# openclimatefix/skillful_nowcasting

Hardware: AMD Instinct MI355X
Metric: radar frames/sec (G+D step) 4->18 @256^2 (higher is better)
Workload: dtype mixed (fp32 tensors + accumulate; bf16x3 = 2 bf16 planes, 3 MFMAs/product, 16-bit products; discriminator forward bf16x6); 1 GPU; DGMR.training_step paper: forecast_steps=18, output_shape=256, latent_channels=768, context_channels=384, generation_steps=6, H=W=256; per_gpu_batch=16, global_batch=16, parallelism=dp1

## Files before the change

skillful_nowcasting_amd/csrc/conv.hip:

```cpp
#include <cstdlib>
#include <cstring>
#include <map>
#include <mutex>
#include <string>
#include <vector>

#include "conv_bf16.h"
#include "conv_device.h"
#include "conv_launch.h"
#include "conv_stem4.h"

namespace {

template <int BM, int BN, int BK, int WM, int WN>
__global__ __launch_bounds__(64 * WM * WN) void conv_igemm_kernel(const dgmr_conv_args p, const int M, const int Ktot,
                                                                   const int kt_per_split) {
    constexpr int NT = 64 * WM * WN;
    constexpr int LD = BK + 4;
    constexpr int KQ = BK / 4;
    constexpr int RPP = NT / KQ;
    constexpr int AP = BM / RPP, BP = BN / RPP;
    constexpr int TM = BM / WM / 32, TN = BN / WN / 32;
    static_assert(AP >= 1 && BP >= 1 && TM >= 1 && TN >= 1, "bad tile");
    static_assert(BM % RPP == 0 && BN % RPP == 0, "bad tile");
// ... 1013 lines not shown
    float a = 0.f;
    if (c < Cout) {
        int r = l;
        for (; r + 28 < nrows; r += 32) {
            float v[8];
#pragma unroll
            for (int k = 0; k < 8; ++k) v[k] = rows[(size_t)(r + 4 * k) * Cout + c];
#pragma unroll
            for (int k = 0; k < 8; ++k) a += v[k];
        }
        for (; r < nrows; r += 4) a += rows[(size_t)r * Cout + c];
    }
    part[l][col] = a;
    __syncthreads();
    if (l == 0 && c < Cout) bias_grad[c] += (part[0][col] + part[1][col]) + (part[2][col] + part[3][col]);
}
static inline int colsum_rows_for(int64_t M) { return (int)std::max<int64_t>(1, std::min<int64_t>(1024, M / 512)); }

static bool wgrad_ws() { return g_tune_wgrad_window != 1; }
static const bool g_wgrad_psplit = []() {
    const char* e = getenv("DGMR_WGRAD_PSPLIT");
    return !(e && e[0] == '0');
}();
static bool wgrad_uses_window(const dgmr_wgrad_args* a) {
    const bool k2d = a->KD == 1 && a->D == 1, k3d = a->KD == 3 && a->D >= 1 && !a->upsample && wgrad_ws();
    return g_precision != 0 && g_tune_wgrad_window != 0 && (k2d || k3d) && a->KH == 3 && a->KW == 3 &&
           ((a->W % 32 == 0 && a->H % 2 == 0) || (a->W == 16 && a->H % 4 == 0));
}
static int wgrad_window_tw_shift(const dgmr_wgrad_args* a) { return a->W % 32 == 0 ? 5 : 4; }
static const bool g_wgrad_phases = []() {
    const char* e = getenv("DGMR_WGRAD_PHASES");
    return !(e && e[0] == '0');
}();
static bool wgrad_by_phases(const dgmr_wgrad_args* a) {
    if (!((g_tune_wgrad_window == 4 || (g_tune_wgrad_window < 0 && g_wgrad_phases)) && a->upsample && a->KD == 1 && a->D == 1 && a->KH == 3 && a->KW == 3 &&
          (g_precision == 1 || g_precision == 2) && a->H % 2 == 0 && a->W % 2 == 0))
        return false;
    const int h = a->H / 2, w = a->W / 2;
    return (w % 32 == 0 && h % 2 == 0) || (w == 16 && h % 4 == 0);
}

extern "C" int dgmr_conv_wgrad_plan(dgmr_wgrad_args* a) {
    DGMR_CHECK_ARG(a && a->N > 0 && a->Cin > 0 && a->Cout > 0, "dgmr_conv_wgrad_plan: bad args");
    const int groups = a->groups < 1 ? 1 : a->groups;
    DGMR_CHECK_ARG(a->N % groups == 0, "dgmr_conv_wgrad_plan: N=%d not divisible by groups=%d", a->N, groups);
    const int64_t M = (int64_t)a->N * a->D * a->H * a->W;
    if (!wgrad_uses_window(a)) {
        a->nsplit = dgmr_conv_wgrad_nsplit((int)M, a->Cout, a->KD * a->KH * a->KW * a->Cin, groups);
        a->bias_rows = std::max(a->nsplit, colsum_rows_for(M));
        return 0;
    }
    const int per_slab = ((a->Cin + 31) / 32) * (a->Cout % 96 == 0 ? a->Cout / 96 : (a->Cout + 63) / 64);
    const bool phases = wgrad_by_phases(a);
    const int64_t tiles_per_group = (int64_t)(a->N / groups) * a->D * ((int64_t)a->H * a->W / (phases ? 256 : 64));
    int64_t per = 512 / ((int64_t)per_slab * groups);
    per = std::min<int64_t>(per, tiles_per_group / 2);
    per = std::max<int64_t>(per, 1);
    if (wgrad_ws()) per = std::max<int64_t>(1, std::min<int64_t>(256 / ((int64_t)per_slab * groups), tiles_per_group / 2));
    a->nsplit = (int)std::min<int64_t>(per * groups, 4096) * (phases ? 4 : 1);
    a->bias_rows = std::max(a->nsplit, colsum_rows_for(M));
    return 0;
}

extern "C" int dgmr_conv_wgrad(const dgmr_wgrad_args* a, void* stream) {
    DGMR_CHECK_ARG(a && a->x && a->dy && a->partial, "dgmr_conv_wgrad: null pointer");
    DGMR_CHECK_ARG(a->Cin % 4 == 0 && a->Cout % 4 == 0, "dgmr_conv_wgrad: Cin=%d Cout=%d must be multiples of 4", a->Cin,
                   a->Cout);
    DGMR_CHECK_ARG(a->nsplit >= 1, "dgmr_conv_wgrad: nsplit=%d", a->nsplit);
// ... 11 lines not shown
    DGMR_CHECK_ARG(!bias_rows_mode || a->bias_rows >= std::max(a->nsplit, colsum_rows_for(M64)),
                   "dgmr_conv_wgrad: bias_rows=%d (dgmr_conv_wgrad_plan fills it in)", a->bias_rows);
    hipStream_t s_ = (hipStream_t)stream;
    auto bias_rows_begin = [&](int rows) { (void)hipMemsetAsync(a->bias_partial, 0, sizeof(float) * (size_t)rows * a->Cout, s_); };
    auto bias_rows_finish = [&](int rows) {
        hipLaunchKernelGGL(bias_rows_finish_kernel, dim3((a->Cout + 63) / 64), dim3(256), 0, s_, a->bias_partial, rows, a->Cout, a->bias_grad);
    };
    auto bias_by_colsum = [&]() {
        const int rows = colsum_rows_for(M64);
        hipLaunchKernelGGL(colsum_rows_kernel, dim3(rows), dim3(256), 0, s_, a->dy, a->bias_partial, M64, a->Cout, rows);
        bias_rows_finish(rows);
    };
    const int M = (int)M64, Ktot = a->KD * a->KH * a->KW * a->Cin;
    const int spg = a->nsplit / groups, rows_per_group = M / groups;
    int rows = (rows_per_group + spg - 1) / spg;
    rows = (rows + 31) / 32 * 32;
    hipStream_t s = (hipStream_t)stream;
    const int kt = (Ktot + 127) / 128;
    const int wclass = a->Cout <= 32 ? V_W32 : (a->Cout <= 64 ? V_W64 : V_W128);
    const uint32_t wdetail = 3u | ((wgrad_uses_window(a) ? (wgrad_ws() ? 2u : 1u) : 0u) << 4) | ((uint32_t)(wclass - V_W128) << 6) |
                             ((a->KD == 3 ? 1u : 0u) << 8) | ((a->upsample ? 1u : 0u) << 9) | ((Ktot == a->Cin ? 1u : 0u) << 10);
    ProfScope ps(wclass, 2.0 * (double)M64 * (double)Ktot * (double)a->Cout, s, 1.0, wdetail);
    if (wgrad_uses_window(a) && wgrad_by_phases(a) && a->nsplit % (4 * groups) == 0) {
        dgmr_wgrad_args q = p;
        q.H = a->H / 2, q.W = a->W / 2, q.upsample = 0;
        const int spg4 = a->nsplit / 4 / groups;
        const int tw_shift = wgrad_window_tw_shift(&q);
        const int tiles_w = q.W >> tw_shift, tiles_hw = (q.H / (64 >> tw_shift)) * tiles_w;
        const int tiles_per_group = (a->N / groups) * tiles_hw;
        const int tiles_per_split = (tiles_per_group + spg4 - 1) / spg4;
        const bool b96 = a->Cout % 96 == 0;
        const dim3 grid((a->Cin + 31) / 32, b96 ? a->Cout / 96 : (a->Cout + 63) / 64, a->nsplit / 4);
        if (bias_rows_mode) bias_rows_begin(a->nsplit);
        for (int ph = 0; ph < 4; ++ph) {
            if (bias_rows_mode) q.bias_grad = a->bias_partial + (size_t)ph * (a->nsplit / 4) * a->Cout, q.bias_stride = a->Cout;
            DGMR_BY_NS(launch_wgrad_window, q, grid, tw_shift, tiles_w, tiles_hw, tiles_per_split, spg4, tiles_per_group,
                       1 | ((g_debug_flags & 16) >> 3) | 4 | 8 | (ph << 16), s);
            DGMR_CHECK_LAUNCH();
        }
        if (bias_rows_mode) bias_rows_finish(a->nsplit);
        return 0;
    }
    if (wgrad_uses_window(a)) {
        const int tw_shift = wgrad_window_tw_shift(a);
        const int tiles_w = a->W >> tw_shift, tiles_hw = (a->H / (64 >> tw_shift)) * tiles_w;
        const int tiles_per_group = (a->N / groups) * a->D * tiles_hw;
        const int tiles_per_split = (tiles_per_group + spg - 1) / spg;
        const bool b96 = a->Cout % 96 == 0;
        const dim3 grid((a->Cin + 31) / 32, b96 ? a->Cout / 96 : (a->Cout + 63) / 64, a->nsplit);
        const bool rows_in_kernel = bias_rows_mode && wgrad_ws();
        if (rows_in_kernel) bias_rows_begin(a->nsplit);
        for (int kd = 0; kd < a->KD; ++kd) {
            dgmr_wgrad_args q = p;
            if (a->KD == 3 && kd != 1) q.bias_grad = nullptr;
            else if (rows_in_kernel) q.bias_grad = a->bias_partial, q.bias_stride = a->Cout;
            else if (bias_rows_mode) q.bias_grad = nullptr;
            DGMR_BY_NS(launch_wgrad_window, q, grid, tw_shift, tiles_w, tiles_hw, tiles_per_split, spg, tiles_per_group,
                       wgrad_ws() ? (1 | ((g_debug_flags & 16) >> 3) | (g_tune_wgrad_window != 2 && g_precision != 3 ? 4 : 0) | ((g_tune_wgrad_window == 5 || !g_wgrad_psplit) ? 32 : 0) | (kd << 8)) : 0, s);
            DGMR_CHECK_LAUNCH();
        }
        if (rows_in_kernel) bias_rows_finish(a->nsplit);
        else if (bias_rows_mode) bias_by_colsum();
        return 0;
    }
    if (bias_rows_mode && g_precision != 0) {
        bias_rows_begin(a->nsplit);
        p.bias_grad = a->bias_partial, p.bias_stride = a->Cout;
    } else if (bias_rows_mode) {
        p.bias_grad = nullptr;
    }
// ... 161 lines not shown
    DGMR_CHECK_LAUNCH();
    return 0;
}

extern "C" int dgmr_split_weights(const float* w, uint16_t* out, int64_t rows, int Cin, int w_cin, int w_coff, int planes,
                                  int64_t plane_stride, void* stream) {
    DGMR_CHECK_ARG(w && out && rows > 0 && Cin > 0 && Cin % 2 == 0, "dgmr_split_weights: bad args (Cin=%d must be even)", Cin);
    DGMR_CHECK_ARG(planes >= 1 && planes <= 3, "dgmr_split_weights: planes=%d (1 .. 3)", planes);
    if (w_cin == 0) {
        w_cin = Cin;
        w_coff = 0;
    }
    DGMR_CHECK_ARG(w_coff >= 0 && w_coff + Cin <= w_cin, "dgmr_split_weights: bad slice");
    const int64_t total = rows * Cin;
    if (plane_stride == 0) plane_stride = total;
    DGMR_CHECK_ARG(plane_stride >= total && plane_stride % 2 == 0, "dgmr_split_weights: plane_stride=%lld < %lld elements", (long long)plane_stride,
                   (long long)total);
    const int blocks = (int)std::min<int64_t>((total / 2 + 255) / 256, 2048);
    hipLaunchKernelGGL(split_weights_kernel, dim3(blocks), dim3(256), 0, (hipStream_t)stream, w, out, total, Cin, w_cin, w_coff, planes,
                       plane_stride);
    DGMR_CHECK_LAUNCH();
    return 0;
}

extern "C" int dgmr_set_precision(int mode) {
    DGMR_CHECK_ARG(mode >= 0 && mode <= 3, "dgmr_set_precision: mode %d (0 f32, 1 bf16x3, 2 bf16, 3 bf16x6)", mode);
    g_precision = mode;
    return 0;
}
extern "C" int dgmr_get_precision(void) { return g_precision; }

extern "C" int dgmr_conv_tune(int variant, int ksplit, int window, int wgrad_window) {
    DGMR_CHECK_ARG(variant >= -1 && variant <= V_F128x32 && ksplit >= -1 && window >= -1 && window <= 7 && wgrad_window >= -1 &&
                       wgrad_window <= 5,
                   "dgmr_conv_tune: variant %d ksplit %d window %d wgrad_window %d", variant, ksplit, window, wgrad_window);
    g_tune_variant = variant;
    g_tune_ksplit = ksplit;
    g_tune_window = window;
    g_tune_wgrad_window = wgrad_window;
    return 0;
}

extern "C" int dgmr_debug_flags(int flags) {
    DGMR_CHECK_ARG(flags >= 0 && flags <= 8191 && !(flags & 4), "dgmr_debug_flags: %d", flags);
    g_debug_flags = flags;
    return 0;
}

extern "C" int dgmr_profile_enable(int on) {
    std::lock_guard<std::mutex> lk(g_prof_mu);
    g_prof_on = on != 0;
    return 0;
}

extern "C" int dgmr_profile_variants(void) { return V_COUNT; }
extern "C" const char* dgmr_profile_variant_name(int v) { return (v >= 0 && v < V_COUNT) ? kVariantNames[v] : ""; }

extern "C" int dgmr_profile_collect(double* total_ms, double* total_flops, int64_t* launches, int n) {
    return dgmr_profile_collect2(total_ms, total_flops, nullptr, launches, n);
}

static std::string prof_detail_name(int variant, uint32_t d) {
    static const char* const prec[] = {"f32", "bf16x3", "bf16", "bf16x6"};
    char b[160];
    const int kind = d & 15;
    const char* pr = prec[(d >> 28) & 3];
    if (kind == 1) {
        static const int bn[] = {48, 64, 96, 128, 16, 0, 0, 0};
        static const char* const mode[] = {"plain", "phase", "pooled", "phase4"};
        snprintf(b, sizeof b, "win3x3<bn%d,%dpx>%s%s%s%s %s %s", bn[(d >> 4) & 7], (d >> 8) & 1 ? 256 : 128, (d >> 13) & 1 ? " reg-staged" : "",
                 (d >> 11) & 1 ? " 3d" : "", (d >> 14) & 1 ? " gru" : "", (d >> 15) & 1 ? " ws" : "", mode[(d >> 9) & 3], (d >> 12) & 1 ? "small(<1024wg)" : "big");
    } else if (kind == 2) {
        snprintf(b, sizeof b, "%s%s%s%s%s %s", kVariantNames[variant], (d >> 8) & 1 ? " splitk" : "", (d >> 9) & 1 ? " 1x1" : "",
                 (d >> 11) & 1 ? " 3d" : "", (d >> 14) & 1 ? " gru" : "", (d >> 12) & 1 ? "small(<1024wg)" : "big");
    } else if (kind == 5) {
        snprintf(b, sizeof b, "conv1x1 stream (%s class)", kVariantNames[variant]);
    } else if (kind == 4) {
// ... 60 lines not shown
```

skillful_nowcasting_amd/csrc/conv_launch.h:

```cpp
#pragma once
#include "common.h"

#define DGMR_HIDDEN __attribute__((visibility("hidden")))

enum { V_F128x128 = 0, V_F64x64, V_F128x96, V_F128x64, V_F128x32, V_W128, V_W64, V_W32, V_WIN128, V_WIN96, V_WIN64, V_COUNT };

struct WinPlan {
    int tw_shift, g_shift, tiles_w, tiles_hw, bnw, grid_x;
    bool big, glds;
    bool ws;
    int ws_ups;
    bool pair;
};

namespace dgmr_tu {

inline int ns_of_precision(int prec) { return prec == 1 ? 3 : (prec == 2 ? 1 : 6); }

#define DGMR_TU_DECLARE(NS)                                                                                                          \
    DGMR_HIDDEN int launch_window_ns##NS(const dgmr_conv_args& p, const WinPlan& wp, bool phases, int tune_window, hipStream_t s);   \
    DGMR_HIDDEN int launch_gemm_ns##NS(int variant, const dgmr_conv_args& p, int M, int Ktot, int kt_per_split, dim3 grid,           \
                                       hipStream_t s);                                                                               \
    DGMR_HIDDEN int launch_wgrad_window_ns##NS(const dgmr_wgrad_args& p, dim3 grid, int tw_shift, int tiles_w, int tiles_hw,         \
                                               int tiles_per_split, int splits_per_group, int tiles_per_group, int ws,         \
                                               hipStream_t s);                                                                        \
    DGMR_HIDDEN int launch_wgrad_gemm_ns##NS(const dgmr_wgrad_args& p, int bi, dim3 grid, int M, int Ktot, int rows_per_split,       \
                                             int splits_per_group, int rows_per_group, hipStream_t s);
DGMR_TU_DECLARE(1)
DGMR_TU_DECLARE(3)
DGMR_TU_DECLARE(6)
#undef DGMR_TU_DECLARE
DGMR_HIDDEN int launch_conv1x1_ns1(const dgmr_conv_args& p, int M, int rows_per_sample, hipStream_t s);
DGMR_HIDDEN int launch_conv1x1_ns3(const dgmr_conv_args& p, int M, int rows_per_sample, hipStream_t s);

#define DGMR_TU_DECLARE_WS(NS, MODE) \
    DGMR_HIDDEN int launch_window_ws_ns##NS##_m##MODE(const dgmr_conv_args& p, const WinPlan& wp, int grid, hipStream_t s);
DGMR_TU_DECLARE_WS(1, 0)
DGMR_TU_DECLARE_WS(1, 1)
DGMR_TU_DECLARE_WS(1, 2)
DGMR_TU_DECLARE_WS(3, 0)
DGMR_TU_DECLARE_WS(3, 1)
DGMR_TU_DECLARE_WS(3, 2)
#undef DGMR_TU_DECLARE_WS

}

#define DGMR_TU_CAT_(a, b) a##b
#define DGMR_TU_CAT(a, b) DGMR_TU_CAT_(a, b)
```

skillful_nowcasting_amd/csrc/tu_wgrad.hip:

```cpp
#include "conv_launch.h"
#include "wgrad_win.h"
#include "wgrad_ws.h"

#ifndef DGMR_NS
#error "compile with -DDGMR_NS=1|3|6"
#endif

namespace dgmr_tu {

int DGMR_TU_CAT(launch_wgrad_window_ns, DGMR_NS)(const dgmr_wgrad_args& p, dim3 grid, int tw_shift, int tiles_w, int tiles_hw,
                                                 int tiles_per_split, int splits_per_group, int tiles_per_group, int ws, hipStream_t s) {
    constexpr int NS = DGMR_NS;
    const bool b96 = p.Cout % 96 == 0;
    if (ws) {
#define DGMR_WGS(BI_, TWS_)                                                                                                      \
    do {                                                                                                                         \
        if constexpr (NS != 6) {                                                                                                 \
            if (ws & 8) {                  \
                hipLaunchKernelGGL((conv_wgrad_ws_kernel<BI_, NS, TWS_, 4, true>), dim3(grid.x * grid.y * grid.z), dim3(512), 0, s, p,     \
                                   tiles_w, tiles_hw, tiles_per_split, splits_per_group, tiles_per_group, ws & 0xff, 0, (ws >> 16) & 3, 4); \
                break;                                                                                                           \
            }                                                                                                                    \
            if (ws & 4) {                                                                                                        \
                hipLaunchKernelGGL((conv_wgrad_ws_kernel<BI_, NS, TWS_, 4>), dim3(grid.x * grid.y * grid.z), dim3(512), 0, s, p, tiles_w, \
                                   tiles_hw, tiles_per_split, splits_per_group, tiles_per_group, ws & 0xff, (ws >> 8) & 0xff);   \
                break;                                                                                                           \
            }                                                                                                                    \
        }                                                                                                                        \
        hipLaunchKernelGGL((conv_wgrad_ws_kernel<BI_, NS, TWS_, 3>), dim3(grid.x * grid.y * grid.z), dim3(448), 0, s, p, tiles_w,    \
                           tiles_hw, tiles_per_split, splits_per_group, tiles_per_group, ws & 0xff, (ws >> 8) & 0xff);           \
    } while (0)
        bool done = false;
        if constexpr (NS != 6) {
            if (p.Cout <= 48 && (ws & 4) && !(ws & 8) && !(ws & 32)) {
                if (tw_shift == 5)
                    hipLaunchKernelGGL((conv_wgrad_ws_kernel<48, NS, 5, 4, false, true>), dim3(grid.x * grid.y * grid.z), dim3(512), 0, s, p, tiles_w,
                                       tiles_hw, tiles_per_split, splits_per_group, tiles_per_group, ws & 0x1f, (ws >> 8) & 0xff);
                else
                    hipLaunchKernelGGL((conv_wgrad_ws_kernel<48, NS, 4, 4, false, true>), dim3(grid.x * grid.y * grid.z), dim3(512), 0, s, p, tiles_w,
                                       tiles_hw, tiles_per_split, splits_per_group, tiles_per_group, ws & 0x1f, (ws >> 8) & 0xff);
                done = true;
            }
        }
        if (done) return 0;
        if (b96) {
            if (tw_shift == 5) DGMR_WGS(96, 5);
            else DGMR_WGS(96, 4);
        } else {
            if (tw_shift == 5) DGMR_WGS(64, 5);
            else DGMR_WGS(64, 4);
// ... 33 lines not shown
```

skillful_nowcasting_amd/csrc/wgrad_ws.h:

```cpp
#pragma once
#include "conv_bf16.h"

namespace {

typedef short s16x4 __attribute__((ext_vector_type(4)));
typedef short s16x8 __attribute__((ext_vector_type(8)));
typedef __attribute__((address_space(3))) s16x4 lds_s16x4;

__device__ __forceinline__ s16x4 lds_read_tr(const uint32_t* p) {
#if defined(__HIP_DEVICE_COMPILE__)
    return __builtin_amdgcn_ds_read_tr16_b64_v4i16((lds_s16x4*)p);
#else
    (void)p;
    return (s16x4){0, 0, 0, 0};
#endif
}
__device__ __forceinline__ bf16x8_t tr_fragment(const uint32_t* p, int row4_dwords) {
    const s16x4 lo = lds_read_tr(p), hi = lds_read_tr(p + row4_dwords);
    const s16x8 v = {lo[0], lo[1], lo[2], lo[3], hi[0], hi[1], hi[2], hi[3]};
    return __builtin_bit_cast(bf16x8_t, v);
}

constexpr int ws_gcd(int a, int b) { return b == 0 ? a : ws_gcd(b, a % b); }

template <int READS, int M, int I>
__device__ __forceinline__ void ws_interleave() {
    if constexpr (I < M) {
        __builtin_amdgcn_sched_group_barrier(0x008, 1, 0);
        constexpr int N = (READS * (I + 1)) / M - (READS * I) / M;
        if constexpr (N > 0) __builtin_amdgcn_sched_group_barrier(0x100, N, 0);
        ws_interleave<READS, M, I + 1>();
    }
}

template <int BI, int NS, int TWS, int MW = 3, bool PHASE = false, bool PSPLIT = false>
__global__ __launch_bounds__(MW * 64 + 256) void conv_wgrad_ws_kernel(const dgmr_wgrad_args p, const int tiles_w, const int tiles_hw,
                                                           const int tiles_per_split, const int splits_per_group,
                                                           const int tiles_per_group, const int dbg, const int kd, const int ph = 0,
                                                           const int slab_mul = 1) {
    static_assert(!PHASE || MW == 4, "phase mode: four matrix waves");
    const int ppy = PHASE ? ph >> 1 : 0, ppx = PHASE ? ph & 1 : 0;
    constexpr int NP = planes_of<NS>::value;
    constexpr int CK = 32, CB = BI / 32;
    constexpr int TW = 1 << TWS, TH = 64 >> TWS;
    constexpr int HTW = TW + 2, HTH = TH + 2;
    constexpr int HPIX = HTH * HTW;
    constexpr int XROW = CK / 2;
    constexpr int YROW = 48;
    constexpr int XPL = HPIX * XROW, YPL = MW == 4 ? 64 * (BI / 2) : 64 * YROW;
    constexpr int BUF = NP * (XPL + YPL);
    constexpr int NL = 256;
    constexpr int XITEMS = HPIX * 8, YQ = BI / 4, YITEMS = 64 * YQ;
    constexpr int XP = (XITEMS + NL - 1) / NL, YP = YITEMS / NL;
    constexpr int BSN = NL % YQ == 0 ? 1 : YQ / ws_gcd(NL % YQ, YQ);
    static_assert(BI == 64 || BI == 96 || (BI == 48 && PSPLIT), "BI");
    static_assert(!PSPLIT || (MW == 4 && !PHASE && BI == 48 && NP <= 2), "pixel-split tile");
    constexpr int NACC4 = 9 * 3 * 4;
    constexpr int RED_DW = ((NL % (BI / 4) == 0 ? 1 : (BI / 4) / ws_gcd(NL % (BI / 4), BI / 4)) * NL * 4);
    constexpr int EXCH_DW = PSPLIT ? 2 * NACC4 * 64 : 0;
    static_assert(TWS == 5 || TWS == 4, "tile width");
    static_assert(YITEMS % NL == 0 && YP % BSN == 0, "dY items per loader thread");

    __shared__ __attribute__((aligned(16))) uint32_t smem[(2 * BUF > RED_DW + EXCH_DW) ? 2 * BUF : RED_DW + EXCH_DW];

    const int tid = threadIdx.x, lane = tid & 63;
    const int wid = __builtin_amdgcn_readfirstlane(tid >> 6);
    const int n_chunks = (p.Cin + CK - 1) / CK, n_cot = (p.Cout + BI - 1) / BI;
    const int total = gridDim.x, xcd = blockIdx.x & 7, per_xcd = total >> 3, rem = total & 7;
    const int wg = xcd * per_xcd + min(xcd, rem) + (blockIdx.x >> 3);
    const int chunk = wg % n_chunks, wg2 = wg / n_chunks;
    const int slab = wg2 / n_cot, co0 = (wg2 - slab * n_cot) * BI;
    const int grp = slab / splits_per_group;
    const int t_begin = grp * tiles_per_group + (slab - grp * splits_per_group) * tiles_per_split;
    const int t_end = min((grp + 1) * tiles_per_group, t_begin + tiles_per_split);
    const int nt = max(t_end - t_begin, 0);
    const bool want_bias = p.bias_grad && chunk == 0;
    float* red = reinterpret_cast<float*>(smem);

    if (wid >= MW) {
        const int lt = tid - MW * 64;
        const int xq = lt & 7;
        const int xci = chunk * CK + xq * 4;
        const bool xc_ok = xci < p.Cin;
        const int us = (!PHASE && p.upsample) ? 1 : 0;
        const int Hs = p.H >> us, Ws = p.W >> us;
        const f32x4 zero4 = {0.f, 0.f, 0.f, 0.f};
        int xrel[XP];
        uint32_t yrel[YP];
        unsigned m_all = 0, m_top = 0, m_bot = 0, m_left = 0, m_right = 0, y_ok = 0;
#pragma unroll
        for (int i = 0; i < XP; ++i) {
            const int idx = lt + i * NL;
            const int pix = idx >> 3;
            const int pr = pix / HTW, pc = pix - pr * HTW;
            xrel[i] = (((pr - 1) >> us) * Ws + ((pc - 1) >> us)) * p.Cin + xci;
            const unsigned bit = 1u << i;
            m_all |= (idx < XITEMS && xc_ok) ? bit : 0u;
            m_top |= pr == 0 ? bit : 0u;
            m_bot |= pr == HTH - 1 ? bit : 0u;
            m_left |= pc == 0 ? bit : 0u;
            m_right |= pc == HTW - 1 ? bit : 0u;
        }
#pragma unroll
        for (int i = 0; i < YP; ++i) {
            const int idx = lt + i * NL;
            const int pix = idx / YQ, q = idx - pix * YQ;
            const int co = co0 + q * 4;
            yrel[i] = PHASE ? (uint32_t)((pix >> TWS) * 4 * p.W + (pix & (TW - 1)) * 2) * p.Cout + min(co, p.Cout - 4)
                            : (uint32_t)((pix >> TWS) * p.W + (pix & (TW - 1))) * p.Cout + min(co, p.Cout - 4);
            y_ok |= co < p.Cout ? 1u << i : 0u;
        }
        int cn = t_begin / tiles_hw, ch0, cw0, left = nt - 1;
        {
            const int trem = t_begin - cn * tiles_hw;
            const int th = trem / tiles_w;
            ch0 = th * TH;
            cw0 = (trem - th * tiles_w) << TWS;
        }
        const int Dp = p.D, dshift = p.KD == 3 ? kd - 1 : 0;
        int cd = cn % Dp;
        const float relu_floor = (p.pre_a || p.pre_relu) ? 0.f : -__builtin_inff();
        f32x4 sx[2][XP], sy[2][YP], sa[2], sb[2], bsum[BSN];
        unsigned xm[2] = {0, 0};
#pragma unroll
        for (int e = 0; e < 2; ++e) sa[e] = (f32x4){1.f, 1.f, 1.f, 1.f}, sb[e] = zero4;
#pragma unroll
        for (int i = 0; i < BSN; ++i) bsum[i] = zero4;

        auto issue = [&](auto set_c) {
            constexpr int E = decltype(set_c)::value;
            const uint32_t xb = (((uint32_t)(cn + dshift) * Hs + (ch0 >> us)) * Ws + (cw0 >> us)) * p.Cin;
            const bool plane_ok = (unsigned)(cd + dshift) < (unsigned)Dp;
            const unsigned kill = (ch0 == 0 ? m_top : 0u) | (ch0 + TH >= p.H ? m_bot : 0u) | (cw0 == 0 ? m_left : 0u) | (cw0 + TW >= p.W ? m_right : 0u);
            const unsigned m = plane_ok ? m_all & ~kill : 0u;
            xm[E] = m;
#pragma unroll
            for (int i = 0; i < XP; ++i) sx[E][i] = *reinterpret_cast<const f32x4*>(p.x + (((m >> i) & 1u) ? xb + (uint32_t)xrel[i] : 0u));
            if (p.pre_a) {
                const uint32_t g = xc_ok ? (uint32_t)(cn / Dp / p.pre_group) * p.Cin + xci : 0u;
                sa[E] = *reinterpret_cast<const f32x4*>(p.pre_a + g);
                sb[E] = *reinterpret_cast<const f32x4*>(p.pre_b + g);
            }
            const float* yb = PHASE ? p.dy + (((size_t)cn * 2 * p.H + 2 * ch0 + ppy) * 2 * p.W + 2 * cw0 + ppx) * p.Cout
                                    : p.dy + (((size_t)cn * p.H + ch0) * p.W + cw0) * p.Cout;
#pragma unroll
            for (int i = 0; i < YP; ++i) sy[E][i] = *reinterpret_cast<const f32x4*>(yb + yrel[i]);
            if (left > 0) {
                --left;
                cw0 += TW;
                if (cw0 >= p.W) {
                    cw0 = 0;
                    ch0 += TH;
                    if (ch0 >= p.H) {
                        ch0 = 0;
                        ++cn;
                        cd = cd + 1 == Dp ? 0 : cd + 1;
                    }
                }
            }
        };
        auto store = [&](auto set_c, bool live) {
            constexpr int E = decltype(set_c)::value;
            uint32_t* Xs = smem + E * BUF + (MW == 4 ? (xq >> 2) * (HPIX * 8) + (lt >> 3) * 8 + (xq & 3) * 2 : lt * 2);
            uint32_t* Ys = smem + E * BUF + NP * XPL;
            const unsigned m = xm[E];
#pragma unroll
            for (int i = 0; i < XP; ++i) {
                if (i == XP - 1 && XITEMS % NL != 0 && lt + i * NL >= XITEMS) continue;
                f32x4 v = sx[E][i];
#pragma unroll
                for (int c = 0; c < 4; ++c) v[c] = fmaxf(fmaf(v[c], sa[E][c], sb[E][c]), relu_floor);
                v = ((m >> i) & 1u) ? v : zero4;
                u32x2 pl[NP];
                split_planes4<NP>(v, pl);
#pragma unroll
                for (int q = 0; q < NP; ++q) *reinterpret_cast<u32x2*>(Xs + q * XPL + i * (MW == 4 ? NL : NL * 2)) = pl[q];
            }
#pragma unroll
            for (int i = 0; i < YP; ++i) {
                const int idx = lt + i * NL;
                const int pix = idx / YQ, q = idx - pix * YQ;
                const f32x4 v = ((y_ok >> i) & 1u) ? sy[E][i] : zero4;
                if (want_bias && live) bsum[i % BSN] += v;
                u32x2 pl[NP];
                split_planes4<NP>(v, pl);
#pragma unroll
                for (int k = 0; k < NP; ++k)
                    *reinterpret_cast<u32x2*>(Ys + k * YPL + (MW == 4 ? (q >> 2) * (64 * 8) + pix * 8 + (q & 3) * 2 : pix * YROW + q * 2)) = pl[k];
            }
        };
        using set0 = std::integral_constant<int, 0>;
        using set1 = std::integral_constant<int, 1>;
        if (nt > 0) {
            issue(set0{});
            issue(set1{});
            store(set0{}, true);
            issue(set0{});
            __syncthreads();
            for (int t = 0; t < nt; t += 2) {
                store(set1{}, t + 1 < nt);
                issue(set1{});
                __syncthreads();
                store(set0{}, t + 2 < nt);
                issue(set0{});
                __syncthreads();
            }
        } else {
            __syncthreads();
        }
        if (want_bias) {
#pragma unroll
            for (int i = 0; i < BSN; ++i) *reinterpret_cast<f32x4*>(red + (i * NL + lt) * 4) = bsum[i];
        }
        if (want_bias || PSPLIT) __syncthreads();
    } else {
        if constexpr (MW == 4) {
            constexpr int CBH = PSPLIT ? 3 : BI / 32;
            const int cih = wid & 1, coh = PSPLIT ? 0 : wid >> 1;
            const int psh = PSPLIT ? wid >> 1 : 0;
            constexpr int NT = PHASE ? 4 : 9;
            f32x4 acc[NT][CBH];
#pragma unroll
            for (int t = 0; t < NT; ++t)
#pragma unroll
                for (int c = 0; c < CBH; ++c) acc[t][c] = (f32x4){0.f, 0.f, 0.f, 0.f};
            const int tg = lane >> 4, ti = lane & 15;
            const int py_lane = 16 * (tg >> 1) + 4 * (tg & 1) + (ti >> 2);
            const int px_lane = (TWS == 5 ? 16 * (tg >> 1) : (tg >> 1) * HTW) + 4 * (tg & 1) + (ti >> 2);
            const int seg = (ti & 3) * 2;
            auto compute = [&](int buf) {
                const uint32_t* Xs = smem + buf * BUF + cih * (HPIX * 8) + px_lane * 8 + seg;
                const uint32_t* Ys = smem + buf * BUF + NP * XPL + coh * CBH * (64 * 8) + py_lane * 8 + seg;
                auto fetch_x = [&](int ks, int pl, bf16x8_t (&dst)[NT]) {
#pragma unroll
                    for (int t = 0; t < NT; ++t) {
                        const int hp = PHASE ? ((TWS == 5 ? ks : 2 * ks) + ppy + (t >> 1)) * HTW + ppx + (t & 1)
                                             : ((TWS == 5 ? ks : 2 * ks) + t / 3) * HTW + t % 3;
                        dst[t] = tr_fragment(Xs + pl * XPL + hp * 8, 8 * 8);
                    }
                };
                auto fetch_y = [&](int ks, int pl, bf16x8_t (&dst)[CBH]) {
#pragma unroll
                    for (int c = 0; c < CBH; ++c) dst[c] = tr_fragment(Ys + pl * YPL + c * (64 * 8) + ks * 32 * 8, 8 * 8);
                };
                auto mm = [&](const bf16x8_t (&y)[CBH], const bf16x8_t (&x)[NT]) {
#pragma unroll
                    for (int t = 0; t < NT; ++t)
#pragma unroll
                        for (int c = 0; c < CBH; ++c) acc[t][c] = __builtin_amdgcn_mfma_f32_16x16x32_bf16(y[c], x[t], acc[t][c], 0, 0, 0);
                };
                constexpr int M = NT * CBH, RX = 2 * NT, RY = CBH * 2, RX0 = PHASE ? 4 : 6;
                if constexpr (PSPLIT) {
                    if constexpr (NP == 2) {
                        bf16x8_t y0[CBH], y1[CBH], x0[NT], x1[NT];
                        fetch_y(psh, 0, y0), fetch_x(psh, 1, x1);
                        __builtin_amdgcn_sched_group_barrier(0x100, RY + RX0, 0);
                        fetch_y(psh, 1, y1), fetch_x(psh, 0, x0);
                        mm(y0, x1);
                        ws_interleave<RX - RX0 + RX + RY, M, 0>();
                        mm(y1, x0);
                        __builtin_amdgcn_sched_group_barrier(0x008, M, 0);
                        mm(y0, x0);
                        __builtin_amdgcn_sched_group_barrier(0x008, M, 0);
                    } else {
                        bf16x8_t xf[NT], yf[CBH];
                        fetch_y(psh, 0, yf), fetch_x(psh, 0, xf);
                        mm(yf, xf);
                    }
                } else if constexpr (NP == 2) {
                    bf16x8_t y0[2][CBH], x0[NT], x1[NT], y1[CBH];
                    fetch_y(0, 0, y0[0]), fetch_x(0, 1, x1);
                    __builtin_amdgcn_sched_group_barrier(0x100, RY + RX0, 0);
#pragma unroll
                    for (int ks = 0; ks < 2; ++ks) {
                        const int e = ks & 1;
                        fetch_y(ks, 1, y1), fetch_x(ks, 0, x0);
                        mm(y0[e], x1);
                        if (ks == 0) ws_interleave<RX - RX0 + RX + RY, M, 0>();
                        else ws_interleave<RX + RY, M, 0>();
                        if (ks < 1) fetch_x(ks + 1, 1, x1), fetch_y(ks + 1, 0, y0[e ^ 1]);
                        mm(y1, x0);
                        if (ks < 1) ws_interleave<RX + RY, M, 0>();
                        else __builtin_amdgcn_sched_group_barrier(0x008, M, 0);
                        mm(y0[e], x0);
                        __builtin_amdgcn_sched_group_barrier(0x008, M, 0);
                    }
                } else {
                    static_assert(NP == 1, "four matrix waves: bf16 and bf16x3 only (bf16x6 needs 144 fragment registers)");
                    bf16x8_t xf[2][NT], yf[2][CBH];
                    fetch_y(0, 0, yf[0]), fetch_x(0, 0, xf[0]);
                    fetch_y(1, 0, yf[1]), fetch_x(1, 0, xf[1]);
                    mm(yf[0], xf[0]);
                    mm(yf[1], xf[1]);
                }
            };
            __builtin_amdgcn_s_setprio(1);
            __syncthreads();
            for (int t = 0; t < nt; t += 2) {
                if (!(dbg & 2)) compute(0);
                __syncthreads();
                if (t + 1 < nt && !(dbg & 2)) compute(1);
                __syncthreads();
            }
            if constexpr (PSPLIT) {
                float* ex = reinterpret_cast<float*>(smem) + RED_DW + cih * (NACC4 * 64) + lane;
                if (psh == 1) {
#pragma unroll
                    for (int t = 0; t < NT; ++t)
#pragma unroll
                        for (int c = 0; c < CBH; ++c)
#pragma unroll
                            for (int r = 0; r < 4; ++r) ex[((t * CBH + c) * 4 + r) * 64] = acc[t][c][r];
                }
                __syncthreads();
                if (psh == 0) {
#pragma unroll
                    for (int t = 0; t < NT; ++t)
#pragma unroll
                        for (int c = 0; c < CBH; ++c)
#pragma unroll
                            for (int r = 0; r < 4; ++r) acc[t][c][r] += ex[((t * CBH + c) * 4 + r) * 64];
                }
            }
            const int Ktot = 9 * p.KD * p.Cin, tap0 = (p.KD == 3 ? kd : 0) * 9;
            float* out = p.partial + ((size_t)slab * slab_mul + (PHASE ? ph : 0)) * p.Cout * Ktot;
            const int ci = chunk * CK + cih * 16 + (lane & 15);
            if (ci < p.Cin && psh == 0) {
#pragma unroll
                for (int c = 0; c < CBH; ++c)
#pragma unroll
                    for (int r = 0; r < 4; ++r) {
                        const int co = co0 + (coh * CBH + c) * 16 + 4 * (lane >> 4) + r;
                        if (co >= p.Cout) continue;
#pragma unroll
                        for (int t = 0; t < 9; ++t) {
                            float v;
                            if constexpr (PHASE) {
                                const int a = (t / 3 + 1 - ppy) >> 1, b = (t % 3 + 1 - ppx) >> 1;
                                const float va0 = b ? acc[1][c][r] : acc[0][c][r], va1 = b ? acc[3][c][r] : acc[2][c][r];
                                v = a ? va1 : va0;
                            } else {
                                v = acc[t][c][r];
                            }
                            out[(size_t)co * Ktot + (tap0 + t) * p.Cin + ci] = v;
                        }
                    }
            }
        } else {
            f32x16 acc[CB * 3];
    #pragma unroll
            for (int a = 0; a < CB * 3; ++a)
    #pragma unroll
                for (int r = 0; r < 16; ++r) acc[a][r] = 0.f;
            const int tg = lane >> 4, ti = lane & 15;
            const int k_lane = 8 * (tg >> 1) + (ti >> 2);
            const int col_lane = 16 * (tg & 1) + 4 * (ti & 3);
            auto compute = [&](int buf) {
                const uint32_t* Xs = smem + buf * BUF;
                const uint32_t* Ys = Xs + NP * XPL;
                auto fetch_x = [&](int kk, int pl, bf16x8_t (&dst)[3]) {
                    const int hp0 = (((kk * 16) >> TWS) + wid) * HTW + ((kk * 16) & (TW - 1));
                    const uint32_t* xb = Xs + pl * XPL + (hp0 + k_lane) * XROW + (col_lane >> 1);
    #pragma unroll
                    for (int d = 0; d < 3; ++d) dst[d] = tr_fragment(xb + d * XROW, 4 * XROW);
                };
                auto fetch_y = [&](int kk, int pl, bf16x8_t (&dst)[CB]) {
                    const uint32_t* yb = Ys + pl * YPL + (kk * 16 + k_lane) * YROW + (col_lane >> 1);
    #pragma unroll
                    for (int c = 0; c < CB; ++c) dst[c] = tr_fragment(yb + c * 16, 4 * YROW);
                };
                auto mm = [&](const bf16x8_t (&y)[CB], const bf16x8_t (&x)[3]) {
    #pragma unroll
                    for (int c = 0; c < CB; ++c)
    #pragma unroll
                        for (int d = 0; d < 3; ++d) acc[c * 3 + d] = __builtin_amdgcn_mfma_f32_32x32x16_bf16(y[c], x[d], acc[c * 3 + d], 0, 0, 0);
                };
                auto interleave = [&](auto reads_c) { ws_interleave<decltype(reads_c)::value, CB * 3, 0>(); };
                if constexpr (NP == 2) {
                    constexpr int RX = 3 * 2, RY = CB * 2;
// ... 29 lines not shown
    #pragma unroll
                        for (int pl = 0; pl < NP; ++pl) fetch_x(kk, pl, xf[pl]), fetch_y(kk, pl, yf[pl]);
                        for_each_product<NP>([&](auto qa, auto qb) { mm(yf[qa], xf[qb]); });
                    }
                }
            };
            __builtin_amdgcn_s_setprio(1);
            __syncthreads();
            for (int t = 0; t < nt; t += 2) {
                if (!(dbg & 2)) compute(0);
                __syncthreads();
                if (t + 1 < nt && !(dbg & 2)) compute(1);
                __syncthreads();
            }
            const int Ktot = 9 * p.KD * p.Cin, tap0 = (p.KD == 3 ? kd : 0) * 9;
            float* out = p.partial + (size_t)slab * p.Cout * Ktot;
            const int ci = chunk * CK + (lane & 31);
            if (ci < p.Cin) {
    #pragma unroll
                for (int c = 0; c < CB; ++c)
    #pragma unroll
                    for (int r = 0; r < 16; ++r) {
                        const int co = co0 + c * 32 + (r & 3) + 8 * (r >> 2) + 4 * (lane >> 5);
                        if (co >= p.Cout) continue;
    #pragma unroll
                        for (int d = 0; d < 3; ++d) out[(size_t)co * Ktot + (tap0 + wid * 3 + d) * p.Cin + ci] = acc[c * 3 + d][r];
                    }
            }
        }
        if (want_bias) {
            if (!PSPLIT) __syncthreads();
            if (tid < BI && co0 + tid < p.Cout) {
                const int q = tid >> 2, comp = tid & 3;
                float total = 0.f;
#pragma unroll
                for (int i = 0; i < BSN; ++i)
                    for (int l = ((q - i * NL) % YQ + YQ) % YQ; l < NL; l += YQ) total += red[(i * NL + l) * 4 + comp];
                atomicAdd(p.bias_grad + (size_t)slab * p.bias_stride + co0 + tid, total);
            }
        }
    }
}

}
```

Baseline: 463.5 radar frames/s.

## Pair column-parity phases in upsample wgrad window kernel to share X tile

For the phase-decomposed weight gradient of upsampled 3x3 convolutions, one launch now handles both column parities of a row phase. The kernel loads the shared input X tile once, stages two dY images, keeps two accumulator sets, and writes both phase outputs and bias partials. This halves the launches (four down to two) and the X loads and plane splitting they repeat. In exchange it doubles dY shared memory, accumulator registers and reduction space, which may lower occupancy. It is on by default through an env flag, and tune value 6 disables the pairing.

```diff
diff --git a/skillful_nowcasting_amd/csrc/conv.hip b/skillful_nowcasting_amd/csrc/conv.hip
--- a/skillful_nowcasting_amd/csrc/conv.hip
+++ b/skillful_nowcasting_amd/csrc/conv.hip
@@ -1069,8 +1069,13 @@
     const char* e = getenv("DGMR_WGRAD_PHASES");
     return !(e && e[0] == '0');
 }();
+static const bool g_wgrad_phase_pair = []() {
+    const char* e = getenv("DGMR_WGRAD_PHASE_PAIR");
+    return !(e && e[0] == '0');
+}();
 static bool wgrad_by_phases(const dgmr_wgrad_args* a) {
-    if (!((g_tune_wgrad_window == 4 || (g_tune_wgrad_window < 0 && g_wgrad_phases)) && a->upsample && a->KD == 1 && a->D == 1 && a->KH == 3 && a->KW == 3 &&
+    const bool tuned = g_tune_wgrad_window == 4 || g_tune_wgrad_window == 6;
+    if (!((tuned || (g_tune_wgrad_window < 0 && g_wgrad_phases)) && a->upsample && a->KD == 1 && a->D == 1 && a->KH == 3 && a->KW == 3 &&
           (g_precision == 1 || g_precision == 2) && a->H % 2 == 0 && a->W % 2 == 0))
         return false;
     const int h = a->H / 2, w = a->W / 2;
@@ -1148,10 +1153,13 @@
         const bool b96 = a->Cout % 96 == 0;
         const dim3 grid((a->Cin + 31) / 32, b96 ? a->Cout / 96 : (a->Cout + 63) / 64, a->nsplit / 4);
         if (bias_rows_mode) bias_rows_begin(a->nsplit);
-        for (int ph = 0; ph < 4; ++ph) {
-            if (bias_rows_mode) q.bias_grad = a->bias_partial + (size_t)ph * (a->nsplit / 4) * a->Cout, q.bias_stride = a->Cout;
+        const bool pair = g_tune_wgrad_window == 4 || (g_tune_wgrad_window < 0 && g_wgrad_phase_pair);
+        const int parity_rows = (a->nsplit / 4) * a->Cout;
+        for (int ph = 0; ph < 4; ph += pair ? 2 : 1) {
+            if (pair && ph && (g_debug_flags & 8192)) break;
+            if (bias_rows_mode) q.bias_grad = a->bias_partial + (size_t)ph * parity_rows, q.bias_stride = a->Cout;
             DGMR_BY_NS(launch_wgrad_window, q, grid, tw_shift, tiles_w, tiles_hw, tiles_per_split, spg4, tiles_per_group,
-                       1 | ((g_debug_flags & 16) >> 3) | 4 | 8 | (ph << 16), s);
+                       1 | ((g_debug_flags & 16) >> 3) | 4 | 8 | (ph << 16) | (pair ? 1 << 18 : 0), s, bias_rows_mode ? parity_rows : 0);
             DGMR_CHECK_LAUNCH();
         }
         if (bias_rows_mode) bias_rows_finish(a->nsplit);
@@ -1379,7 +1387,7 @@
 
 extern "C" int dgmr_conv_tune(int variant, int ksplit, int window, int wgrad_window) {
     DGMR_CHECK_ARG(variant >= -1 && variant <= V_F128x32 && ksplit >= -1 && window >= -1 && window <= 7 && wgrad_window >= -1 &&
-                       wgrad_window <= 5,
+                       wgrad_window <= 6,
                    "dgmr_conv_tune: variant %d ksplit %d window %d wgrad_window %d", variant, ksplit, window, wgrad_window);
     g_tune_variant = variant;
     g_tune_ksplit = ksplit;
@@ -1389,7 +1397,7 @@
 }
 
 extern "C" int dgmr_debug_flags(int flags) {
-    DGMR_CHECK_ARG(flags >= 0 && flags <= 8191 && !(flags & 4), "dgmr_debug_flags: %d", flags);
+    DGMR_CHECK_ARG(flags >= 0 && flags <= 16383 && !(flags & 4), "dgmr_debug_flags: %d", flags);
     g_debug_flags = flags;
     return 0;
 }
diff --git a/skillful_nowcasting_amd/csrc/conv_launch.h b/skillful_nowcasting_amd/csrc/conv_launch.h
--- a/skillful_nowcasting_amd/csrc/conv_launch.h
+++ b/skillful_nowcasting_amd/csrc/conv_launch.h
@@ -23,7 +23,7 @@
                                        hipStream_t s);                                                                               \
     DGMR_HIDDEN int launch_wgrad_window_ns##NS(const dgmr_wgrad_args& p, dim3 grid, int tw_shift, int tiles_w, int tiles_hw,         \
                                                int tiles_per_split, int splits_per_group, int tiles_per_group, int ws,         \
-                                               hipStream_t s);                                                                        \
+                                               hipStream_t s, int pair_bias = 0);                                                     \
     DGMR_HIDDEN int launch_wgrad_gemm_ns##NS(const dgmr_wgrad_args& p, int bi, dim3 grid, int M, int Ktot, int rows_per_split,       \
                                              int splits_per_group, int rows_per_group, hipStream_t s);
 DGMR_TU_DECLARE(1)
diff --git a/skillful_nowcasting_amd/csrc/tu_wgrad.hip b/skillful_nowcasting_amd/csrc/tu_wgrad.hip
--- a/skillful_nowcasting_amd/csrc/tu_wgrad.hip
+++ b/skillful_nowcasting_amd/csrc/tu_wgrad.hip
@@ -9,13 +9,20 @@
 namespace dgmr_tu {
 
 int DGMR_TU_CAT(launch_wgrad_window_ns, DGMR_NS)(const dgmr_wgrad_args& p, dim3 grid, int tw_shift, int tiles_w, int tiles_hw,
-                                                 int tiles_per_split, int splits_per_group, int tiles_per_group, int ws, hipStream_t s) {
+                                                 int tiles_per_split, int splits_per_group, int tiles_per_group, int ws, hipStream_t s,
+                                                 int pair_bias) {
     constexpr int NS = DGMR_NS;
     const bool b96 = p.Cout % 96 == 0;
     if (ws) {
 #define DGMR_WGS(BI_, TWS_)                                                                                                      \
     do {                                                                                                                         \
         if constexpr (NS != 6) {                                                                                                 \
+            if ((ws & 8) && (ws & (1 << 18))) {      \
+                hipLaunchKernelGGL((conv_wgrad_ws_kernel<BI_, NS, TWS_, 4, true, false, true>), dim3(grid.x * grid.y * grid.z), dim3(512), 0, \
+                                   s, p, tiles_w, tiles_hw, tiles_per_split, splits_per_group, tiles_per_group, ws & 0xff, 0,   \
+                                   (ws >> 16) & 2, 4, pair_bias);                                                                \
+                break;                                                                                                           \
+            }                                                                                                                    \
             if (ws & 8) {                  \
                 hipLaunchKernelGGL((conv_wgrad_ws_kernel<BI_, NS, TWS_, 4, true>), dim3(grid.x * grid.y * grid.z), dim3(512), 0, s, p,     \
                                    tiles_w, tiles_hw, tiles_per_split, splits_per_group, tiles_per_group, ws & 0xff, 0, (ws >> 16) & 3, 4); \
diff --git a/skillful_nowcasting_amd/csrc/wgrad_ws.h b/skillful_nowcasting_amd/csrc/wgrad_ws.h
--- a/skillful_nowcasting_amd/csrc/wgrad_ws.h
+++ b/skillful_nowcasting_amd/csrc/wgrad_ws.h
@@ -33,13 +33,15 @@
     }
 }
 
-template <int BI, int NS, int TWS, int MW = 3, bool PHASE = false, bool PSPLIT = false>
+template <int BI, int NS, int TWS, int MW = 3, bool PHASE = false, bool PSPLIT = false, bool PAIR = false>
 __global__ __launch_bounds__(MW * 64 + 256) void conv_wgrad_ws_kernel(const dgmr_wgrad_args p, const int tiles_w, const int tiles_hw,
                                                            const int tiles_per_split, const int splits_per_group,
                                                            const int tiles_per_group, const int dbg, const int kd, const int ph = 0,
-                                                           const int slab_mul = 1) {
+                                                           const int slab_mul = 1, const int pair_bias = 0) {
     static_assert(!PHASE || MW == 4, "phase mode: four matrix waves");
-    const int ppy = PHASE ? ph >> 1 : 0, ppx = PHASE ? ph & 1 : 0;
+    static_assert(!PAIR || PHASE, "pair: both column parities of a phase launch");
+    constexpr int NPAR = PAIR ? 2 : 1;
+    const int ppy = PHASE ? ph >> 1 : 0, ppx = (PHASE && !PAIR) ? ph & 1 : 0;
     constexpr int NP = planes_of<NS>::value;
     constexpr int CK = 32, CB = BI / 32;
     constexpr int TW = 1 << TWS, TH = 64 >> TWS;
@@ -48,7 +50,8 @@
     constexpr int XROW = CK / 2;
     constexpr int YROW = 48;
     constexpr int XPL = HPIX * XROW, YPL = MW == 4 ? 64 * (BI / 2) : 64 * YROW;
-    constexpr int BUF = NP * (XPL + YPL);
+    constexpr int YIMG = NP * YPL;
+    constexpr int BUF = NP * XPL + NPAR * YIMG;
     constexpr int NL = 256;
     constexpr int XITEMS = HPIX * 8, YQ = BI / 4, YITEMS = 64 * YQ;
     constexpr int XP = (XITEMS + NL - 1) / NL, YP = YITEMS / NL;
@@ -56,7 +59,8 @@
     static_assert(BI == 64 || BI == 96 || (BI == 48 && PSPLIT), "BI");
     static_assert(!PSPLIT || (MW == 4 && !PHASE && BI == 48 && NP <= 2), "pixel-split tile");
     constexpr int NACC4 = 9 * 3 * 4;
-    constexpr int RED_DW = ((NL % (BI / 4) == 0 ? 1 : (BI / 4) / ws_gcd(NL % (BI / 4), BI / 4)) * NL * 4);
+    constexpr int RED1 = ((NL % (BI / 4) == 0 ? 1 : (BI / 4) / ws_gcd(NL % (BI / 4), BI / 4)) * NL * 4);
+    constexpr int RED_DW = NPAR * RED1;
     constexpr int EXCH_DW = PSPLIT ? 2 * NACC4 * 64 : 0;
     static_assert(TWS == 5 || TWS == 4, "tile width");
     static_assert(YITEMS % NL == 0 && YP % BSN == 0, "dY items per loader thread");
@@ -120,12 +124,12 @@
         const int Dp = p.D, dshift = p.KD == 3 ? kd - 1 : 0;
         int cd = cn % Dp;
         const float relu_floor = (p.pre_a || p.pre_relu) ? 0.f : -__builtin_inff();
-        f32x4 sx[2][XP], sy[2][YP], sa[2], sb[2], bsum[BSN];
+        f32x4 sx[2][XP], sy[2][NPAR * YP], sa[2], sb[2], bsum[NPAR][BSN];
         unsigned xm[2] = {0, 0};
 #pragma unroll
         for (int e = 0; e < 2; ++e) sa[e] = (f32x4){1.f, 1.f, 1.f, 1.f}, sb[e] = zero4;
 #pragma unroll
-        for (int i = 0; i < BSN; ++i) bsum[i] = zero4;
+        for (int i = 0; i < NPAR * BSN; ++i) bsum[i / BSN][i % BSN] = zero4;
 
         auto issue = [&](auto set_c) {
             constexpr int E = decltype(set_c)::value;
@@ -143,8 +147,9 @@
             }
             const float* yb = PHASE ? p.dy + (((size_t)cn * 2 * p.H + 2 * ch0 + ppy) * 2 * p.W + 2 * cw0 + ppx) * p.Cout
                                     : p.dy + (((size_t)cn * p.H + ch0) * p.W + cw0) * p.Cout;
-#pragma unroll
-            for (int i = 0; i < YP; ++i) sy[E][i] = *reinterpret_cast<const f32x4*>(yb + yrel[i]);
+            const float* const yb1 = yb + p.Cout;
+#pragma unroll
+            for (int i = 0; i < NPAR * YP; ++i) sy[E][i] = *reinterpret_cast<const f32x4*>((i < YP ? yb : yb1) + yrel[i % YP]);
             if (left > 0) {
                 --left;
                 cw0 += TW;
@@ -177,16 +182,29 @@
                 for (int q = 0; q < NP; ++q) *reinterpret_cast<u32x2*>(Xs + q * XPL + i * (MW == 4 ? NL : NL * 2)) = pl[q];
             }
 #pragma unroll
-            for (int i = 0; i < YP; ++i) {
+            for (int j = 0; j < NPAR * YP; ++j) {
+                const int i = j % YP, par = j / YP;
                 const int idx = lt + i * NL;
                 const int pix = idx / YQ, q = idx - pix * YQ;
-                const f32x4 v = ((y_ok >> i) & 1u) ? sy[E][i] : zero4;
-                if (want_bias && live) bsum[i % BSN] += v;
+                const f32x4 v = ((y_ok >> i) & 1u) ? sy[E][j] : zero4;
+                if (!PAIR && want_bias && live) bsum[0][i % BSN] += v;
                 u32x2 pl[NP];
                 split_planes4<NP>(v, pl);
 #pragma unroll
                 for (int k = 0; k < NP; ++k)
-                    *reinterpret_cast<u32x2*>(Ys + k * YPL + (MW == 4 ? (q >> 2) * (64 * 8) + pix * 8 + (q & 3) * 2 : pix * YROW + q * 2)) = pl[k];
+                    *reinterpret_cast<u32x2*>(Ys + par * YIMG + k * YPL + (MW == 4 ? (q >> 2) * (64 * 8) + pix * 8 + (q & 3) * 2 : pix * YROW + q * 2)) = pl[k];
+            }
+            if constexpr (PAIR) {
+                if (want_bias && live) {
+#pragma unroll
+                    for (int j = 0; j < NPAR * BSN; ++j) {
+                        const int par = j / BSN, slot = j % BSN;
+                        f32x4 b = bsum[par][slot];
+#pragma unroll
+                        for (int i = slot; i < YP; i += BSN) b += ((y_ok >> i) & 1u) ? sy[E][par * YP + i] : zero4;
+                        bsum[par][slot] = b;
+                    }
+                }
             }
         };
         using set0 = std::integral_constant<int, 0>;
@@ -210,7 +228,7 @@
         }
         if (want_bias) {
 #pragma unroll
-            for (int i = 0; i < BSN; ++i) *reinterpret_cast<f32x4*>(red + (i * NL + lt) * 4) = bsum[i];
+            for (int i = 0; i < NPAR * BSN; ++i) *reinterpret_cast<f32x4*>(red + (i / BSN) * RED1 + ((i % BSN) * NL + lt) * 4) = bsum[i / BSN][i % BSN];
         }
         if (want_bias || PSPLIT) __syncthreads();
     } else {
@@ -219,22 +237,28 @@
             const int cih = wid & 1, coh = PSPLIT ? 0 : wid >> 1;
             const int psh = PSPLIT ? wid >> 1 : 0;
             constexpr int NT = PHASE ? 4 : 9;
-            f32x4 acc[NT][CBH];
-#pragma unroll
-            for (int t = 0; t < NT; ++t)
-#pragma unroll
-                for (int c = 0; c < CBH; ++c) acc[t][c] = (f32x4){0.f, 0.f, 0.f, 0.f};
+            f32x4 accs[NPAR][NT][CBH];
+#pragma unroll
+            for (int a = 0; a < NPAR; ++a)
+#pragma unroll
+                for (int t = 0; t < NT; ++t)
+#pragma unroll
+                    for (int c = 0; c < CBH; ++c) accs[a][t][c] = (f32x4){0.f, 0.f, 0.f, 0.f};
+            auto& acc = accs[0];
             const int tg = lane >> 4, ti = lane & 15;
             const int py_lane = 16 * (tg >> 1) + 4 * (tg & 1) + (ti >> 2);
             const int px_lane = (TWS == 5 ? 16 * (tg >> 1) : (tg >> 1) * HTW) + 4 * (tg & 1) + (ti >> 2);
             const int seg = (ti & 3) * 2;
-            auto compute = [&](int buf) {
+            auto compute = [&](int buf, auto par_c) {
+                constexpr int PAR = decltype(par_c)::value;
+                auto& acc = accs[PAR];
+                const int pxx = PAIR ? PAR : ppx;
                 const uint32_t* Xs = smem + buf * BUF + cih * (HPIX * 8) + px_lane * 8 + seg;
-                const uint32_t* Ys = smem + buf * BUF + NP * XPL + coh * CBH * (64 * 8) + py_lane * 8 + seg;
+                const uint32_t* Ys = smem + buf * BUF + NP * XPL + PAR * YIMG + coh * CBH * (64 * 8) + py_lane * 8 + seg;
                 auto fetch_x = [&](int ks, int pl, bf16x8_t (&dst)[NT]) {
 #pragma unroll
                     for (int t = 0; t < NT; ++t) {
-                        const int hp = PHASE ? ((TWS == 5 ? ks : 2 * ks) + ppy + (t >> 1)) * HTW + ppx + (t & 1)
+                        const int hp = PHASE ? ((TWS == 5 ? ks : 2 * ks) + ppy + (t >> 1)) * HTW + pxx + (t & 1)
                                              : ((TWS == 5 ? ks : 2 * ks) + t / 3) * HTW + t % 3;
                         dst[t] = tr_fragment(Xs + pl * XPL + hp * 8, 8 * 8);
                     }
@@ -294,12 +318,20 @@
                     mm(yf[1], xf[1]);
                 }
             };
+            using par0 = std::integral_constant<int, 0>;
+            using par1 = std::integral_constant<int, 1>;
             __builtin_amdgcn_s_setprio(1);
             __syncthreads();
             for (int t = 0; t < nt; t += 2) {
-                if (!(dbg & 2)) compute(0);
-                __syncthreads();
-                if (t + 1 < nt && !(dbg & 2)) compute(1);
+                if (!(dbg & 2)) {
+                    compute(0, par0{});
+                    if constexpr (PAIR) compute(0, par1{});
+                }
+                __syncthreads();
+                if (t + 1 < nt && !(dbg & 2)) {
+                    compute(1, par0{});
+                    if constexpr (PAIR) compute(1, par1{});
+                }
                 __syncthreads();
             }
             if constexpr (PSPLIT) {
@@ -323,28 +355,33 @@
                 }
             }
             const int Ktot = 9 * p.KD * p.Cin, tap0 = (p.KD == 3 ? kd : 0) * 9;
-            float* out = p.partial + ((size_t)slab * slab_mul + (PHASE ? ph : 0)) * p.Cout * Ktot;
             const int ci = chunk * CK + cih * 16 + (lane & 15);
             if (ci < p.Cin && psh == 0) {
 #pragma unroll
-                for (int c = 0; c < CBH; ++c)
-#pragma unroll
-                    for (int r = 0; r < 4; ++r) {
-                        const int co = co0 + (coh * CBH + c) * 16 + 4 * (lane >> 4) + r;
-                        if (co >= p.Cout) continue;
-#pragma unroll
-                        for (int t = 0; t < 9; ++t) {
-                            float v;
-                            if constexpr (PHASE) {
-                                const int a = (t / 3 + 1 - ppy) >> 1, b = (t % 3 + 1 - ppx) >> 1;
-                                const float va0 = b ? acc[1][c][r] : acc[0][c][r], va1 = b ? acc[3][c][r] : acc[2][c][r];
-                                v = a ? va1 : va0;
-                            } else {
-                                v = acc[t][c][r];
+                for (int par = 0; par < NPAR; ++par) {
+                    auto& acc = accs[par];
+                    const int pxx = PAIR ? par : ppx;
+                    float* out = p.partial + ((size_t)slab * slab_mul + (PHASE ? ph + par : 0)) * p.Cout * Ktot;
+#pragma unroll
+                    for (int c = 0; c < CBH; ++c)
+#pragma unroll
+                        for (int r = 0; r < 4; ++r) {
+                            const int co = co0 + (coh * CBH + c) * 16 + 4 * (lane >> 4) + r;
+                            if (co >= p.Cout) continue;
+#pragma unroll
+                            for (int t = 0; t < 9; ++t) {
+                                float v;
+                                if constexpr (PHASE) {
+                                    const int a = (t / 3 + 1 - ppy) >> 1, b = (t % 3 + 1 - pxx) >> 1;
+                                    const float va0 = b ? acc[1][c][r] : acc[0][c][r], va1 = b ? acc[3][c][r] : acc[2][c][r];
+                                    v = a ? va1 : va0;
+                                } else {
+                                    v = acc[t][c][r];
+                                }
+                                out[(size_t)co * Ktot + (tap0 + t) * p.Cin + ci] = v;
                             }
-                            out[(size_t)co * Ktot + (tap0 + t) * p.Cin + ci] = v;
                         }
-                    }
+                }
             }
         } else {
             f32x16 acc[CB * 3];
@@ -440,11 +477,14 @@
             if (!PSPLIT) __syncthreads();
             if (tid < BI && co0 + tid < p.Cout) {
                 const int q = tid >> 2, comp = tid & 3;
-                float total = 0.f;
-#pragma unroll
-                for (int i = 0; i < BSN; ++i)
-                    for (int l = ((q - i * NL) % YQ + YQ) % YQ; l < NL; l += YQ) total += red[(i * NL + l) * 4 + comp];
-                atomicAdd(p.bias_grad + (size_t)slab * p.bias_stride + co0 + tid, total);
+#pragma unroll
+                for (int par = 0; par < NPAR; ++par) {
+                    float total = 0.f;
+#pragma unroll
+                    for (int i = 0; i < BSN; ++i)
+                        for (int l = ((q - i * NL) % YQ + YQ) % YQ; l < NL; l += YQ) total += red[par * RED1 + (i * NL + l) * 4 + comp];
+                    atomicAdd(p.bias_grad + (size_t)par * pair_bias + (size_t)slab * p.bias_stride + co0 + tid, total);
+                }
             }
         }
     }
```

Measured after the change: 465.5 radar frames/s (median of 6 runs). About the same (+0.4%).
